# SaeedRahmani/AV-Simulation-at-Intersections

Hardware: AMD Instinct MI355X
Metric: MPC steps/sec (batch x horizon) at N=20 nu=2 (higher is better)
Workload: dtype f64

## Files before the change

### av-simulation-at-intersections_amd/_cabi.py

```python
from __future__ import annotations

import ctypes as C
import os

from .config import MPCConfig

_HERE = os.path.dirname(os.path.abspath(__file__))
LIB_PATH = os.environ.get("JSIM_LIB_PATH") or os.path.join(_HERE, "libjsim_mpc.so")
ABI_VERSION = 2


class JsimCfg(C.Structure):
    _fields_ = [
        ("T", C.c_int32), ("max_iter", C.c_int32),
        ("dt", C.c_double), ("dl", C.c_double), ("L", C.c_double),
        ("w_perp", C.c_double), ("w_para", C.c_double),
        ("R", C.c_double * 2), ("Rd", C.c_double * 2), ("Q_v_yaw", C.c_double * 2),
        ("Qf", C.c_double * 4), ("R_end", C.c_double * 2),
        ("max_dsteer", C.c_double), ("max_accel", C.c_double), ("max_decel", C.c_double),
        ("max_steer", C.c_double), ("max_speed", C.c_double), ("min_speed", C.c_double),
        ("min_ref_speed", C.c_double), ("goal_dis", C.c_double), ("stop_speed", C.c_double),
        ("nx", C.c_int32), ("reserved_", C.c_int32), ("jerk_weight", C.c_double),
    ]


EXPORTS = (
    "jsim_abi_version", "jsim_last_error", "jsim_mpc_create", "jsim_mpc_destroy", "jsim_mpc_set_paths",
    "jsim_mpc_step", "jsim_mpc_step_debug", "jsim_plant_step", "jsim_loop_advance", "jsim_mpc_run_ticks", "jsim_mpc_set_launch_order", "jsim_mpc_get_launch_order", "jsim_mpc_iter_totals",
    "jsim_loop_set_geometry", "jsim_loop_set_obstacle_geometry", "jsim_loop_predict_obstacles", "jsim_loop_pre_tick",
    "jsim_mpc_set_path_speed", "jsim_mpc_set_speed_cutoff", "jsim_mpc_update_cfg", "jsim_mpc_set_ego_config", "jsim_loop_obstacles",
    "jsim_mpc_xref_deviation_goal", "jsim_loop_run_scenario",
    "jsim_loop_set_groups", "jsim_loop_predict_egos", "jsim_loop_run_interacting",
    "jsim_loop_set_traffic", "jsim_loop_set_recorder", "jsim_loop_set_vehicle_shapes",
    "jsim_comm_unique_id", "jsim_comm_init", "jsim_mpc_gather", "jsim_comm_destroy", "jsim_plan_routes",
    "jsim_plan_routes_weighted", "jsim_score_trajectories", "jsim_loop_eval_reasons", "jsim_loop_eval_conflicts",
    "jsim_loop_eval_static", "jsim_loop_summarise_episodes", "jsim_loop_eval_cutoffs", "jsim_loop_fork_state", "jsim_loop_obstacles_at",
    "jsim_loop_eval_gaps",
)

_lib = None


class JsimError(RuntimeError):
    pass


def load() -> C.CDLL:
    global _lib
    if _lib is not None:
        return _lib
    if not os.path.exists(LIB_PATH):
        raise JsimError(
            f"{LIB_PATH} is missing: build it with `python __graft_entry__.py` (hipcc, gfx950). "
            "The MPC path is HIP-only; there is no CPU fallback.")
    lib = C.CDLL(LIB_PATH)
    vp, i32, i64, dbl = C.c_void_p, C.c_int32, C.c_int64, C.c_double
    lib.jsim_abi_version.restype = C.c_int
    lib.jsim_abi_version.argtypes = []
    lib.jsim_last_error.restype = C.c_char_p
    lib.jsim_last_error.argtypes = [vp]
    lib.jsim_mpc_create.restype = C.c_int
    lib.jsim_mpc_create.argtypes = [C.POINTER(JsimCfg), C.c_int, C.POINTER(vp)]
    lib.jsim_mpc_destroy.restype = None
    lib.jsim_mpc_destroy.argtypes = [vp]
    lib.jsim_mpc_set_paths.restype = C.c_int
    lib.jsim_mpc_set_paths.argtypes = [vp, vp, vp, vp, vp, i32]
    lib.jsim_mpc_step.restype = C.c_int
# ... 116 lines not shown
```

### av-simulation-at-intersections_amd/batched.py

```python
from __future__ import annotations

import ctypes as C
from typing import List, Optional, Sequence, Union

import numpy as np
import torch

from . import _cabi
from .config import MPCConfig
from .synth import pack_paths, smooth_yaw_inplace


def _ptr(t: Optional[torch.Tensor]):
    return None if t is None else C.c_void_p(t.data_ptr())


class BatchedMPC:

    def __init__(self, paths: Sequence[np.ndarray], path_id: Union[np.ndarray, Sequence[int]], dl: float,
                 L: float = 2.86, speed: Union[float, np.ndarray] = 30 / 3.6, dt: float = 0.2,
                 T: Optional[int] = None, config: Optional[MPCConfig] = None,
                 device: Union[str, torch.device] = "cuda:0", smooth: bool = True,
                 cv: Optional[Sequence[np.ndarray]] = None):
        self.lib = _cabi.load()
# ... 37 lines not shown
        self.path_id = torch.from_numpy(pid).to(dev)
        full = np.array([self.paths[i].shape[0] for i in pid], dtype=np.int32)
        self.path_len = torch.from_numpy(full.copy()).to(dev)
        self.full_len = torch.from_numpy(full).to(dev)
        sp = np.broadcast_to(np.asarray(speed, dtype=np.float64), (B,)).copy()
        self.speed = torch.from_numpy(sp).to(dev)
        MW = (8 * T + 31) // 32
        spec = [("target_ind", torch.int64, (B,)), ("oa", torch.float64, (B, T)), ("od", torch.float64, (B, T)),
                ("ox", torch.float64, (B, T + 1)), ("oy", torch.float64, (B, T + 1)), ("ov", torch.float64, (B, T + 1)),
                ("oyaw", torch.float64, (B, T + 1)), ("xref", torch.float64, (B, 4, T + 1)), ("di_ai", torch.float64, (B, 2)),
                ("active_mask", torch.int32, (B, MW)), ("status", torch.int32, (B,)), ("n_iter", torch.int32, (B,))]
        self._arena_layout = {}
        nbytes = 0
        for name, dt, shape in spec:
            n = int(np.prod(shape)) * torch.empty((), dtype=dt).element_size()
            self._arena_layout[name] = (nbytes, n, dt, shape)
            nbytes += (n + 7) & ~7
        self._arena = torch.zeros(max(nbytes, 8), dtype=torch.uint8, device=dev)
        for name, (o, n, dt, shape) in self._arena_layout.items():
            setattr(self, name, self._arena[o:o + n].view(dt).view(shape))

    def read_back(self) -> dict:
        host = self._arena.cpu().numpy()
        return {name: host[o:o + n].view(torch.empty((), dtype=dt).numpy().dtype).reshape(shape)
                for name, (o, n, dt, shape) in self._arena_layout.items()}

    def _upload_paths(self):
        cx, cy, cyaw, off = pack_paths(self.paths)
        self._path_off = off
        _cabi.check(self.lib.jsim_mpc_set_paths(self._ctx, cx.ctypes.data, cy.ctypes.data, cyaw.ctypes.data,
                                                off.ctypes.data, len(self.paths)), self._ctx, "jsim_mpc_set_paths")

    def set_path_len(self, path_len: Union[np.ndarray, torch.Tensor]):
        if isinstance(path_len, torch.Tensor):
            pl = path_len.to(device=self.device, dtype=torch.int32)
        else:
            pl = torch.from_numpy(np.ascontiguousarray(path_len, dtype=np.int32)).to(self.device)
        if pl.shape != (self.B,):
            raise ValueError("path_len must have shape [B]")
        if bool((pl < 1).any()) or bool((pl > self.full_len).any()):
            raise ValueError("path_len must satisfy 1 <= path_len[b] <= len(paths[path_id[b]])")
        self.path_len = pl.contiguous()

    def set_speed_cutoff(self, cutoff: Optional[Union[np.ndarray, torch.Tensor]]):
        if cutoff is None:
            self.cv_cut = None
            _cabi.check(self.lib.jsim_mpc_set_speed_cutoff(self._ctx, None), self._ctx, "jsim_mpc_set_speed_cutoff")
            return
# ... 109 lines not shown
```

### av-simulation-at-intersections_amd/csrc/mpc_step_reg.inc

```

template <int CTRL>
__device__ __forceinline__ double dpp_f64(double v)
{
    int lo = __double2loint(v), hi = __double2hiint(v);
    lo = __builtin_amdgcn_update_dpp(0, lo, CTRL, 0xf, 0xf, true);
    hi = __builtin_amdgcn_update_dpp(0, hi, CTRL, 0xf, 0xf, true);
    return __hiloint2double(hi, lo);
}
template <int CTRL>
__device__ __forceinline__ int dpp_i32(int v) { return __builtin_amdgcn_update_dpp(0, v, CTRL, 0xf, 0xf, true); }

#define DPP_QP_1032 0xB1
#define DPP_QP_2301 0x4E
#define DPP_ROW_HALF_MIRROR 0x141
#define DPP_ROW_MIRROR 0x140
#define DPP_ROW_SHR(n) (0x110 + (n))

__device__ __forceinline__ double wsum_dpp(double v)
{
    v += dpp_f64<DPP_QP_1032>(v);
    v += dpp_f64<DPP_QP_2301>(v);
    v += dpp_f64<DPP_ROW_HALF_MIRROR>(v);
    v += dpp_f64<DPP_ROW_MIRROR>(v);
    return (rdlane(v, 0) + rdlane(v, 16)) + (rdlane(v, 32) + rdlane(v, 48));
// ... 181 lines not shown
#endif
#ifndef JSIM_CHUNK_WAITS
#define JSIM_CHUNK_WAITS 15
#endif

#include "loop_pre_tick.inc"

struct PreK {
    PreP pre;
    const double2 *pred_cc_all;
    const double4 *pred_bc_all;
    long long *traj_idx;
    int *prev_len;
    int *path_len_out;
    int speed_cutoff;
    int *cut_io;
    int *col_flag;
    int *pre_status;
    TrafficP traffic;
};

enum { HB_SKIP = 0, HB_SCAN = 1, HB_HBUILD = 2, HB_JBUILD = 3, HB_EXIT = 4 };

__device__ __forceinline__ void jsim_spin_published(const double *val_lds)
{
    const unsigned addr = (unsigned)(__UINTPTR_TYPE__)(__attribute__((address_space(3))) const double *)val_lds;
    int v, cnt, cur;
    asm volatile("s_mov_b32 %1, 0\n"
                 "1:\n\t"
                 "ds_read_b32 %0, %3 offset:4\n\t"
                 "s_waitcnt lgkmcnt(0)\n\t"
                 "v_readfirstlane_b32 %2, %0\n\t"
                 "s_add_u32 %1, %1, 1\n\t"
                 "s_cmp_lg_u32 %2, 0xbff00000\n\t"
                 "s_cbranch_scc1 2f\n\t"
                 "s_cmp_lt_u32 %1, 0x400000\n\t"
                 "s_cbranch_scc1 1b\n"
                 "2:"
                 : "=&v"(v), "=&s"(cnt), "=&s"(cur)
                 : "v"(addr)
                 : "memory", "scc");
}

template <int T, int ROW>
__device__ __forceinline__ void jsim_h_tile_row(const double *tq, double *Hm, int lane, double dt)
{
    constexpr int N = 2 * T, LD = N + 1, TP = T + 2;
    const int kk = lane >> 4, cc = lane & 15;
    double c0[ROW + 1], c1[ROW + 1], p0[ROW + 1], p1[ROW + 1];
    int thr[ROW + 1];
    const bool isd_ = cc & 1;
    const int xrow = (kk < 2 ? (isd_ ? TQ_PB : TQ_PA) : TQ_ONE) * TP, yrow = (kk < 2 ? (isd_ ? TQ_PBP : TQ_PAP) : TQ_ONE) * TP;
    const int w0row = (kk == 0 ? TQ_QXX : kk == 1 ? TQ_QXY : kk == 2 ? TQ_QV : TQ_QYAW) * TP;
    const int w1row = (kk == 0 ? TQ_QXY : kk == 1 ? TQ_QYY : TQ_ZERO) * TP;
#pragma unroll
    for (int c = 0; c <= ROW; ++c) {
        const int col = 16 * c + cc;
        const bool vcol = col < N;
        const int s = vcol ? (col >> 1) : (T - 1);
        const double ks = tq[TQ_KT * TP + s];
        const double coef = vcol ? (isd_ ? ks : dt) : 0.0;
        const double c23 = !vcol ? 0.0 : (kk == 2 ? (isd_ ? 0.0 : dt) : (kk == 3 ? (isd_ ? ks : 0.0) : 0.0));
        c0[c] = kk < 2 ? coef : c23;
        c1[c] = kk < 2 ? coef : 0.0;
// ... 59 lines not shown
template <int T, bool PRE, int WPE, bool HELP = false>
__global__ __launch_bounds__(HELP ? 256 : 64) __attribute__((amdgpu_waves_per_eu(WPE, WPE)))
void mpc_step_reg_kernel(const KP Pin, const TickP K, const PreK Q)
{
    static_assert(!HELP || (WPE == 1 && (2 * T + 15) / 16 <= 4), "helpers: one wave per SIMD, one helper per tile row");
    KP P = Pin;
    if ((int)blockIdx.x >= Pin.B) return;
    const int ego = K.order ? K.order[blockIdx.x] : (int)blockIdx.x;
    if (Pin.pe) jsim_apply_ego_cfg(P, Pin.pe, ego, Pin.T, Pin.dt);
    constexpr int N = 2 * T, NR = 3 * T + 1, LD = N + 1, TP = T + 2, MW = (8 * T + 31) / 32;
    constexpr int NTILE = (N + 15) / 16;
    constexpr bool VS = NR >= 64;
    constexpr int NW = VS ? N : NR;
    static_assert(NW < 64, "register path needs 2T+1 lanes (3T+2 with resident speed rows)");
    constexpr int NP = N + 2;
    constexpr int CHW = VS ? 0 : HELP ? (JSIM_CHUNK_WAITS & ~2) : JSIM_CHUNK_WAITS;
    constexpr int LDC = N + 2, CCH = 16;
    constexpr bool LCA = VS || (WPE == 2 && T > 13);
    constexpr int HLN = LCA ? N * LDC : N * LD + N * LDC;
    constexpr int PREN = PRE ? (int)((sizeof(PreScratch) + 7) / 8) : 0;
    __shared__ __attribute__((aligned(16))) double HL[HLN > PREN ? HLN : PREN];
    double *const Hm = HL;
    constexpr bool HCLR = HELP && !LCA;
    double *const Lc = HL + (LCA ? 0 : N * LD);
    static_assert((N * LD) % 2 == 0, "Lc stays 16-byte aligned");
    __shared__ __attribute__((aligned(16))) double gsv[2 * N];
    __shared__ __attribute__((aligned(16))) double drow12[2 * NP];
    double *const drow = drow12, *const drow2 = drow12 + NP;
    __shared__ __attribute__((aligned(16))) double dzv[NP];
    __shared__ __attribute__((aligned(16))) double vzv[NP];
    __shared__ __attribute__((aligned(16))) double rdv[NP];
    __shared__ __attribute__((aligned(16))) double UV[VS ? 2 : NR + 5];
    constexpr int TQN = (TQ_COUNT * TP + 1) & ~1 ;
    constexpr int SPH = (T + 1) & ~1, SPN = VS ? T * SPH : 0;
    static_assert(!VS || (SPN >= NR + 5 || TQN + 3 * NP >= NR + 5), "uvec fits the shared area");
    __shared__ __attribute__((aligned(16))) double SCR[(TQN + 3 * NP > SPN) ? TQN + 3 * NP : SPN];
    double *const tq = SCR, *const invc = SCR + TQN, *const gvc = SCR + TQN + NP, *const wvc = SCR + TQN + 2 * NP;
    double *const spdump = SCR;
    double *const uvec = VS ? SCR : UV;
    __shared__ unsigned maskw[MW + 1];
    __shared__ int hb_cmd, hb_ilen;
    __shared__ __attribute__((aligned(16))) double Jx[HELP ? 64 * (N + 2) : 2];
    __shared__ long long hb_s0;
    __shared__ double hb_xy[2], hb_rd[HELP ? 12 : 2];
    __shared__ int hb_ri[HELP ? 12 : 2];

    const int lane0 = HELP ? (int)(threadIdx.x & 63) : (int)threadIdx.x;
    const int hwave = HELP ? __builtin_amdgcn_readfirstlane((int)(threadIdx.x >> 6)) : 0;
    if (P.pass > 0 && P.status[ego] != JSIM_OK) return;
    const int it_base = (P.pass > 0 && P.n_iter) ? P.n_iter[ego] : 0;
    int lane = lane0;

    const int pid = P.path_id[ego];
    const long long off = P.poff[pid];
    long long M = P.path_len[ego];
    long long pre_idx = 0;
    int pre_prev = -1, pre_col = 0, pre_st = JSIM_OK, Mfull = 0, pre_cut = -1;
    ObsSlice pre_obs = {0, 0};
    const double2 *pre_othr = nullptr;
    if (PRE) {
        pre_obs = traffic_slice(Q.traffic, ego, Q.pre.n_obs);
        pre_obs.first = uni(pre_obs.first); pre_obs.n = uni(pre_obs.n);
        if (Q.pre.othr) pre_othr = Q.pre.othr + pre_obs.first;
        pre_idx = Q.traj_idx[ego];
// ... 39 lines not shown
                    const double2 p0 = pp[k], p1 = pp[k + 192], p2 = pp[k + 384], p3 = pp[k + 576];
                    HB_INSERT_PT(p0, k) HB_INSERT_PT(p1, k + 192) HB_INSERT_PT(p2, k + 384) HB_INSERT_PT(p3, k + 576)
                }
                for (; k < ilen; k += 192) {
                    const double2 p0 = pp[k];
                    HB_INSERT_PT(p0, k)
                }
#undef HB_INSERT_PT
#pragma unroll
                for (int r = 0; r < 3; ++r) {
                    double v = b0;
                    int id = i0;
                    wargmin_fast(v, id);
                    if (lane0 == 0) { hb_rd[(hwave - 1) * 3 + r] = v; hb_ri[(hwave - 1) * 3 + r] = id; }
                    if (i0 == id) { b0 = b1; i0 = i1; b1 = b2; i1 = i2; b2 = INFINITY; i2 = 0x7fffffff; }
                }
            } else if (cmd == HB_HBUILD) {
                if (hwave == 1 && NTILE > 1) jsim_h_tile_row<T, 1>(tq, Hm, lane0, dt);
                else if (hwave == 2 && NTILE > 2) jsim_h_tile_row<T, 2>(tq, Hm, lane0, dt);
                else if (hwave == 3 && NTILE > 3) jsim_h_tile_row<T, 3>(tq, Hm, lane0, dt);
                if (hwave == 3) { const double gi = jsim_g_own<T>(tq, lane0, dt); if (lane0 < N) gvc[lane0] = gi; }
            } else if (cmd == HB_JBUILD && hwave == 1) {
                double Jr[N];
#define JSIM_J_WAIT(n_) jsim_spin_published(&invc[(n_) - 1])
#include "mpc_step_reg_j.inc"
#undef JSIM_J_WAIT
#pragma unroll
                for (int j = 0; j < N; j += 2) *(double2 *)&Jx[lane0 * (N + 2) + j] = double2{Jr[j], Jr[j + 1]};
            } else if (cmd == HB_JBUILD && HCLR) {
                for (int e = (hwave - 2) * 64 + lane0; e < N * LD; e += 128) Hm[e] = 0.0;
                if (hwave == 2 && lane0 < N) { gsv[2 * lane0] = 1.0; gsv[2 * lane0 + 1] = 0.0; }
                if (hwave == 3 && lane0 < 2) { drow[N + lane0] = 0.0; drow2[N + lane0] = 0.0; dzv[N + lane0] = 0.0; vzv[N + lane0] = 0.0; }
            }
            __syncthreads();
        }
    }
    double wtan;
    {
        double dc = (P.smax < wd_t) ? P.smax : wd_t;
        dc = (-P.smax > dc) ? -P.smax : dc;
        wtan = tan(dc);
    }
    for (int tk = 0; tk < K.n_ticks; ++tk) {
    if (WPE == 2) {
        sx = uni(sx); sy = uni(sy); sv = uni(sv); syaw = uni(syaw); di_prev = uni(di_prev); ai_last = uni(ai_last);
        goal_xy.x = uni(goal_xy.x); goal_xy.y = uni(goal_xy.y); s0 = uni64(s0); age = uni(age);
    }
#define LANE_FENCE() do { lane = lane0; asm volatile("" : "+v"(lane)); __builtin_assume(lane >= 0 && lane < 64); } while (0)
    LANE_FENCE();
    if (PRE) {
        PreScratch &W = *reinterpret_cast<PreScratch *>(HL);
        PreP pre = Q.pre;
        pre.n_obs = pre_obs.n;
        const PreOut o = jsim_pre_tick_ego(pre, Q.pred_cc_all + ((size_t)tk * Q.pre.n_obs + pre_obs.first) * Q.pre.n_steps * 2,
                                           Q.pred_bc_all + (size_t)tk * Q.pre.n_obs + pre_obs.first, pre_othr, W, lane, ego,
                                           off, Mfull, sx, sy, sv, pre_idx, pre_prev);
        pre_st = o.status;
        if (o.status == JSIM_OK) {
            pre_idx = o.idx; pre_col = o.col;
            if (Q.speed_cutoff) pre_cut = o.path_len; else M = o.path_len;
        }
        pre_prev = Q.speed_cutoff ? Mfull : (int)M;
        LDS_SYNC();
        LANE_FENCE();
    }
// ... 277 lines not shown
                        const double hv = 2.0 * acc[a][b][r];
                        Hm[row * LD + col] = hv;
                        if (a != b) Hm[col * LD + row] = hv;
                    }
                }
    }
    LDS_SYNC();
    STAMP(5);
    LANE_FENCE();
    double A[N];
    {
        const int i = lane < N ? lane : 0;
        const int t = i >> 1, c = i & 1;
        const double Rt = (tq[TQ_REND * TP + t] != 0.0) ? (c ? P.Re1 : P.Re0) : (c ? P.R1 : P.R0);
        const double rdc = 2.0 * (c ? P.Rd1 : P.Rd0);
        const int nd = (T >= 2) ? ((t == 0 || t == T - 1) ? 1 : 2) : 0;
        if (lane < N) {
            Hm[i * LD + i] += 2.0 * Rt + nd * rdc;
            if (i + 2 < N) Hm[i * LD + i + 2] -= rdc;
            if (i >= 2) Hm[i * LD + i - 2] -= rdc;
        }
        LDS_SYNC();
#pragma unroll
        for (int j = 0; j < N; ++j) A[j] = Hm[i * LD + j];
    }
    if (P.dbg_g && lane < N) P.dbg_g[(size_t)ego * N + lane] = gi_own;
    if (P.dbg_H && lane < N) {
        double *Hd = P.dbg_H + (size_t)ego * N * N + (size_t)lane * N;
#pragma unroll
        for (int j = 0; j < N; ++j) Hd[j] = A[j];
    }
    const double gmax = wmax_dpp(fabs(gi_own));

    if (lane < N) gvc[lane] = gi_own;
    STAMP(6);
    LANE_FENCE();
    if (HELP) {
        if (lane < N) invc[lane] = -1.0;
        if (lane == 0) hb_cmd = HB_JBUILD;
        __syncthreads();
    }
    {
        JSIM_OPAQUE_ZERO(zc_);
        const double *const LcC = Lc + zc_;
        double inv, tmul;
        {
            if (lane < N) Lc[lane] = A[0];
            double ck = rdlane(A[0], 0);
            if (!(ck > 0.0)) ck = 1e-300;
            inv = fast_rsqrt(ck);
            tmul = A[0] * (inv * inv);
        }
#pragma unroll
        for (int k = 0; k < N; ++k) {
            LDS_SYNC();
            const int j0 = k & ~1;
            const int nch = (N - j0 + CCH - 1) / CCH;
            double2 cb[2][CCH / 2];
#pragma unroll
            for (int j = j0; j < j0 + CCH && j < N; j += 2) cb[0][(j - j0) / 2] = *(const double2 *)&LcC[k * LDC + j];
            if (HELP) __builtin_amdgcn_fence(__ATOMIC_RELEASE, "wavefront");
            if (lane == k) invc[k] = inv;
            const double tk = tmul;
            if (k + 1 < N) {
                JSIM_STAGE();
                if (!(k & 1)) JSIM_PIN_PAIR(cb[0][0]);
                const double cn = ((k + 1) & 1) ? cb[0][(k + 1 - j0) / 2].y : cb[0][(k + 1 - j0) / 2].x;
                A[k + 1] = fma(-tk, cn, A[k + 1]);
                JSIM_PIN(A[k + 1]);
                if (lane >= k + 1 && lane < N) Lc[(k + 1) * LDC + lane] = A[k + 1];
                double ck = rdlane(A[k + 1], k + 1);
                if (!(ck > 0.0)) ck = 1e-300;
                inv = fast_rsqrt(ck);
                tmul = A[k + 1] * (inv * inv);
            }
#pragma unroll
            for (int c = 0; c < nch; ++c) {
                const int h = j0 + c * CCH;
                if (c + 1 < nch) {
#pragma unroll
                    for (int j = h + CCH; j < h + 2 * CCH && j < N; j += 2) cb[(c + 1) & 1][(j - h - CCH) / 2] = *(const double2 *)&LcC[k * LDC + j];
                }
                if ((CHW & 1) && k + 1 < N) jsim_chunk_wait((c + 1 < nch ? ((h + 2 * CCH < N ? h + 2 * CCH : N) - (h + CCH)) / 2 : 0) + (c == 0 ? 2 : 0));
                JSIM_STAGE();
#pragma unroll
                for (int j = h; j < h + CCH && j < N; j += 2) {
                    const double2 c2 = cb[c & 1][(j - h) / 2];
                    if (j > k + 1) { A[j] = fma(-tk, c2.x, A[j]); JSIM_PIN(A[j]); }
                    if (j + 1 > k + 1) { A[j + 1] = fma(-tk, c2.y, A[j + 1]); JSIM_PIN(A[j + 1]); }
                }
                JSIM_STAGE();
            }
        }
    }
    LDS_SYNC();

    STAMP(7);
    LANE_FENCE();
    double Jr[N];
    if (!HELP) {
#define JSIM_J_WAIT(n_) do { } while (0)
#include "mpc_step_reg_j.inc"
#undef JSIM_J_WAIT
    } else {
        __syncthreads();
        hp = 3;
#pragma unroll
        for (int j = 0; j < N; j += 2) { const double2 v2 = *(const double2 *)&Jx[lane * (N + 2) + j]; Jr[j] = v2.x; Jr[j + 1] = v2.y; }
    }
    LDS_SYNC();

    STAMP(8);
    LANE_FENCE();
    double val = 0.0;
    {
        double v0 = 0.0, v1 = 0.0;
        JSIM_OPAQUE_ZERO(zw_);
        const double *const wvW = wvc + zw_;
#pragma unroll
        for (int h = 0; h < N; h += CCH) {
            double2 wb[CCH / 2];
#pragma unroll
            for (int j = h; j < h + CCH && j < N; j += 2) wb[(j - h) / 2] = *(const double2 *)&wvW[j];
            JSIM_STAGE();
#pragma unroll
            for (int j = h; j < h + CCH && j < N; j += 2) {
                v0 = fma(-Jr[j], wb[(j - h) / 2].x, v0);
                v1 = fma(-Jr[j + 1], wb[(j - h) / 2].y, v1);
            }
// ... 465 lines not shown
        }
        if (failed) { status = JSIM_INFEASIBLE; break; }
    }
#undef JSIM_SEARCH
#undef JSIM_SEARCH_A
#undef JSIM_SEARCH_B1
#undef JSIM_SEARCH_B2
#undef JSIM_SEARCH_C

    STAMP(10);
#ifdef JSIM_STAMPS
    if (P.dbg_clk && lane == 0)
        for (int i_ = 0; i_ < 8; ++i_) P.dbg_clk[(size_t)P.B * 16 + (size_t)ego * 8 + i_] = gclk[i_];
#endif
    LANE_FENCE();
    if (status != JSIM_OK) {
        if (tl) { P.oa[(size_t)ego * T + lane] = 0.0; P.od[(size_t)ego * T + lane] = 0.0; }
        wa_t = 0.0; wd_t = 0.0; wtan = 0.0; s0 = tind;
        if (P.amask && lane < MW) P.amask[(size_t)ego * MW + lane] = 0u;
        if (lane == 0) {
            P.status[ego] = status;
            P.target_ind[ego] = tind;
            if (P.n_iter) P.n_iter[ego] = it_base + iters;
            if (K.work) K.work[ego] += (unsigned)iters;
            if (K.iters) K.iters[ego] += (unsigned long long)iters;
        }
        break;
    }
    if (lane < MW) maskw[lane] = 0u;
    if (lane < (VS ? N : NR)) uvec[lane] = val;
    if (VS) {
        const bool evl = lane < N && !(lane & 1);
        const double vsp = fma(dt, wincscan_dpp(evl ? val : 0.0, lane), sv);
        if (evl) uvec[N + (lane >> 1) + 1] = vsp;
        if (lane == 0) uvec[N] = sv;
    }
    if (P.dbg_lam)
        for (int e = lane; e < 8 * T; e += 64) P.dbg_lam[(size_t)ego * 8 * T + e] = 0.0;
    LDS_SYNC();
    {
        const double thr = JSIM_ACT_TOL * fmax(1.0, gmax);
        if (lane < q) {
            if (lam > thr) atomicOr(&maskw[actid >> 5], 1u << (actid & 31));
            if (P.dbg_lam) P.dbg_lam[(size_t)ego * 8 * T + actid] = lam;
        }
        LDS_SYNC();
        if (P.amask && lane < MW) P.amask[(size_t)ego * MW + lane] = maskw[lane];
    }
    {
// ... 7 lines not shown
        const double yt = syaw + wexscan_dpp(kt * dl_, lane);
        const double xt = sx + wexscan_dpp(fma(al, vt, fma(be, yt, ccx)), lane);
        const double yy = sy + wexscan_dpp(fma(alp, vt, fma(bep, yt, ccy)), lane);
        if (tl) { P.oa[(size_t)ego * T + lane] = a; P.od[(size_t)ego * T + lane] = dl_; }
        wa_t = a; wd_t = dl_; s0 = tind;
        if (K.advance || tk + 1 < K.n_ticks) {
            double dc = (P.smax < dl_) ? P.smax : dl_;
            dc = (-P.smax > dc) ? -P.smax : dc;
            wtan = tan(dc);
        }
        a0n = uvec[0]; d0n = uvec[1];
        if (lane <= T) {
            const size_t o = (size_t)ego * (T + 1) + lane;
            if (P.ox) P.ox[o] = xt;
            if (P.oy) P.oy[o] = yy;
            if (P.ov) P.ov[o] = vt;
            if (P.oyaw) P.oyaw[o] = yt;
        }
    }
    if (lane == 0) {
        P.status[ego] = JSIM_OK;
        P.target_ind[ego] = tind;
        if (P.n_iter) P.n_iter[ego] = it_base + iters;
        if (K.work) K.work[ego] += (unsigned)iters;
        if (K.iters) K.iters[ego] += (unsigned long long)iters;
    }
    STAMP(11);
    } while (0);
    if (HELP)
        for (; hp < 3; ++hp) {
            if (lane0 == 0) hb_cmd = HB_SKIP;
            __syncthreads();
            __syncthreads();
        }

    if (K.advance) {
        double di = di_prev, ai;
        if (status == JSIM_OK) { di = d0n; ai = a0n; }
        else ai = P.amin;
        di_prev = di;
        ai_last = ai;
        if (K.hist && lane == 0) {
            const int k = hist_base + tk;
            if (k < K.hist_cap) { K.hist[((size_t)k * P.B + ego) * 2] = di; K.hist[((size_t)k * P.B + ego) * 2 + 1] = ai; }
        }
        if (K.rec && lane == 0 && *K.tick + tk < K.rec_cap)
            jsim_rec_store_dev(K.rec, *K.tick + tk, P.B, ego,
                               status == JSIM_OK ? jsim_xref_deviation(P.pxy[off + s0], P.pyaw[off + s0], sx, sy) : __builtin_nan(""));
        double dc = (P.smax < di) ? P.smax : di;
// ... 18 lines not shown
        const bool done = (isgoal && fabs(sv) <= K.stop_speed) || (age + 1 >= K.max_age);
        if (K.rec && lane == 0) {
            const int k = *K.tick + tk;
            if (k < K.rec_cap)
                jsim_rec_store(K.rec, K.rec_flags, k, P.B, ego, sx, sy, syaw, sv, di, ai,
                               (status == JSIM_OK ? 0 : JSIM_REC_FAILED) | (isgoal && fabs(sv) <= K.stop_speed ? JSIM_REC_GOAL : 0) |
                                   (age + 1 >= K.max_age ? JSIM_REC_AGE : 0));
        }
        if (done) {
            sx = K.x0_spawn[4 * ego]; sy = K.x0_spawn[4 * ego + 1]; sv = K.x0_spawn[4 * ego + 2]; syaw = K.x0_spawn[4 * ego + 3];
            s0 = K.target_spawn[ego];
            wa_t = 0.0; wd_t = 0.0; wtan = 0.0; di_prev = 0.0; ai_last = 0.0; age = 0;
            if (PRE) { pre_idx = 0; pre_prev = -1; }
            if (tl) { P.oa[(size_t)ego * T + lane] = 0.0; P.od[(size_t)ego * T + lane] = 0.0; }
            if (lane == 0) {
                P.target_ind[ego] = s0;
                if (K.n_respawn) atomicAdd(K.n_respawn, 1ull);
            }
        } else {
            age += 1;
        }
    }
    LDS_SYNC();
    }
    if (HELP) {
        if (lane0 == 0) hb_cmd = HB_EXIT;
        __syncthreads();
    }
    if (K.advance && lane == 0) {
        K.x0w[4 * ego] = sx; K.x0w[4 * ego + 1] = sy; K.x0w[4 * ego + 2] = sv; K.x0w[4 * ego + 3] = syaw;
        K.di_ai[2 * ego] = di_prev;
        K.di_ai[2 * ego + 1] = ai_last;
        K.age[ego] = age;
    }
    if (PRE && lane == 0) {
        Q.traj_idx[ego] = pre_idx;
        Q.prev_len[ego] = pre_prev;
        if (Q.speed_cutoff) Q.cut_io[ego] = pre_cut; else Q.path_len_out[ego] = (int)M;
        Q.col_flag[ego] = pre_col;
        Q.pre_status[ego] = pre_st;
    }
}
```

### av-simulation-at-intersections_amd/csrc/mpc_step_reg4.inc

```

__host__ __device__ constexpr int jsim_tile_wave4(int ntile, int a)
{
    return ntile == 5 ? (a == 0 || a == 4 ? 0 : a) : (a & 3);
}

__device__ __forceinline__ double pair_swap(double v)
{
    double r = dpp_f64<DPP_QP_1032>(v);
    asm volatile("" : "+v"(r));
    return r;
}

#ifndef JSIM_REG4_MINW
#define JSIM_REG4_MINW 2
#endif

template <int T, bool PRE>
__global__ __launch_bounds__(256, JSIM_REG4_MINW) void mpc_step_reg4_kernel(const KP P, const TickP K, const PreK Q)
{
    constexpr int N = 2 * T, NH = T, NR = 3 * T + 1, LD = N + 2, TP = T + 2, MW = (8 * T + 31) / 32, NP = N + 2;
    constexpr int NTILE = (N + 15) / 16;
    constexpr int G1 = 31, G2 = 61;
    constexpr int S2 = 64 + (N - G2);
    constexpr int SW = S2 + T + 1;
// ... 62 lines not shown
        Mfull = (int)(gp(Pv.poff)[pid + 1] - off);
        if (Q.speed_cutoff) pre_cut = Q.cut_io[ego];
    }
    const double speed = uni(gp(Pv.speed)[ego]);
    const double dt = uni((double)Pv.dt);
#define tl (lane < T)
    long long s0 = uni64(gp(Pv.target_ind)[ego]);
    double sx = gp(Pv.x0)[4 * ego + 0], sy = gp(Pv.x0)[4 * ego + 1], sv = gp(Pv.x0)[4 * ego + 2], syaw = gp(Pv.x0)[4 * ego + 3];
#define WS_SET(a_, d_) do { if (wave == 0 && tl) { wsv[0][lane] = (a_); wsv[1][lane] = (d_); } } while (0)
#define WS_TAN(d_, out_) do { const double sm_ = Pv.smax; double dc_ = (sm_ < (d_)) ? sm_ : (d_); dc_ = (-sm_ > dc_) ? -sm_ : dc_; out_ = tan(dc_); } while (0)
    {
        double wt0 = 0.0;
        if (wave == 0 && tl) { const double od0 = gp(Pv.od)[(size_t)ego * T + lane]; WS_TAN(od0, wt0); }
        WS_SET(gp(Pv.oa)[(size_t)ego * T + lane], wt0);
    }
    __syncthreads();
    double di_prev = advance ? gp(Kv.di_ai)[2 * ego] : 0.0;
    double ai_last = advance ? gp(Kv.di_ai)[2 * ego + 1] : 0.0;
    int age = advance ? uni(gp(Kv.age)[ego]) : 0;
    const int hist_base = (advance && (Kv.hist || Kv.rec)) ? uni(*gp(Kv.tick)) : 0;
    double2 goal_xy = double2{0.0, 0.0};
    if (advance) { const jsim_d2v gq = ((JSIM_GAS const jsim_d2v *)Pv.pxy)[gp(Pv.poff)[pid + 1] - 1]; goal_xy = double2{uni(gq.x), uni(gq.y)}; }

    for (int tk = 0; tk < n_ticks; ++tk) {
#define LANE_FENCE4() do { unsigned ones_ = ~0u; asm volatile("" : "+s"(ones_)); gl = (wave << 6) | (int)__builtin_amdgcn_mbcnt_hi(ones_, __builtin_amdgcn_mbcnt_lo(ones_, 0u)); asm volatile("" : "+v"(gl)); __builtin_assume(gl >= 0 && gl < 256); lane = gl & 63; } while (0)
    LANE_FENCE4();
    sx = uni(sx); sy = uni(sy); sv = uni(sv); syaw = uni(syaw); di_prev = uni(di_prev); ai_last = uni(ai_last);
    s0 = uni64(s0); M = uni64(M); age = uni(age);
    if (PRE) {
        PreScratch &W = *reinterpret_cast<PreScratch *>(Hm);
        PreP pre = Q.pre;
        pre.n_obs = pre_obs.n;
        const PreOut o = jsim_pre_tick_ego<true>(pre, Q.pred_cc_all + ((size_t)tk * Q.pre.n_obs + pre_obs.first) * Q.pre.n_steps * 2,
                                           Q.pred_bc_all + (size_t)tk * Q.pre.n_obs + pre_obs.first, pre_othr, W, lane, ego,
                                           off, Mfull, sx, sy, sv, pre_idx, pre_prev);
        pre_st = o.status;
        if (o.status == JSIM_OK) {
            pre_idx = o.idx; pre_col = o.col;
            if (Q.speed_cutoff) pre_cut = o.path_len; else M = o.path_len;
        }
        pre_prev = Q.speed_cutoff ? Mfull : (int)M;
        BLOCK_SYNC();
        LANE_FENCE4();
    }
    double a0n = 0.0, d0n = 0.0;
    int status = JSIM_OK;
// ... 989 lines not shown
                    if (slot == dslot) abits &= ~(1u << dbit);
                    JSIM_PIN(abits);
                }
                GSTAMP(7);
            }
        }
        if (failed) { status = JSIM_INFEASIBLE; break; }
    }

#ifdef JSIM_STAMPS
    if (Pv.dbg_clk && gl == 0)
        for (int i_ = 0; i_ < 8; ++i_) Pv.dbg_clk[(size_t)Pv.B * 16 + (size_t)ego * 8 + i_] = gclk[i_];
#endif
    LANE_FENCE4();
    STAMP2(10);
    if (status != JSIM_OK) {
        if (wave == 0 && tl) { gp(Pv.oa)[(size_t)ego * T + lane] = 0.0; gp(Pv.od)[(size_t)ego * T + lane] = 0.0; }
        WS_SET(0.0, 0.0); s0 = tind;
        if (Pv.amask && gl < MW) gp(Pv.amask)[(size_t)ego * MW + gl] = 0u;
        if (gl == 0) {
            gp(Pv.status)[ego] = status;
            gp(Pv.target_ind)[ego] = tind;
            if (Pv.n_iter) gp(Pv.n_iter)[ego] = it_base + iters;
            if (Kv.work) gp(Kv.work)[ego] += (unsigned)iters;
            if (Kv.iters) gp(Kv.iters)[ego] += (unsigned long long)iters;
        }
        break;
    }
    if (gl < MW) maskw[gl] = 0u;
    {
        const int slot_ = gl >> 1;
        if (!(gl & 1)) {
            int jr_ = -1;
            if (slot_ < G1) jr_ = slot_;
            else if (slot_ > G1 && slot_ < G2 + 1) jr_ = slot_ - 1;
            else if (slot_ >= 64 && slot_ < S2) jr_ = slot_ - 3;
            if (jr_ >= 0) uvec[jr_] = val;
            if (slot_ >= S2 && slot_ < SW) uvec[N + slot_ - S2] = val;
        }
    }
    if (Pv.dbg_lam)
        for (int e = gl; e < 8 * T; e += 256) Pv.dbg_lam[(size_t)ego * 8 * T + e] = 0.0;
    BLOCK_SYNC();
    {
        const double thr = JSIM_ACT_TOL * fmax(1.0, gmax);
        if (wave == 0) {
            if (lane < q) {
                if (lam0 > thr) atomicOr(&maskw[act0 >> 5], 1u << (act0 & 31));
                if (Pv.dbg_lam) Pv.dbg_lam[(size_t)ego * 8 * T + act0] = lam0;
// ... 13 lines not shown
        if (tl) { a = uvec[2 * lane]; dl_ = uvec[2 * lane + 1]; }
        const double vt = lane <= T ? uvec[N + lane] : sv;
        const double yt = syaw + wexscan_dpp(kt * dl_, lane);
        const double xt = sx + wexscan_dpp(fma(al, vt, fma(be, yt, ccx)), lane);
        const double yy = sy + wexscan_dpp(fma(alp, vt, fma(bep, yt, ccy)), lane);
        if (wave == 0 && tl) { gp(Pv.oa)[(size_t)ego * T + lane] = a; gp(Pv.od)[(size_t)ego * T + lane] = dl_; }
        double tn = 0.0;
        if (advance || tk + 1 < n_ticks) WS_TAN(dl_, tn);
        p_tn = rdlane(tn, 0);
        WS_SET(a, tn); s0 = tind;
        a0n = uvec[0]; d0n = uvec[1];
        if (wave == 0 && lane <= T) {
            const size_t o = (size_t)ego * (T + 1) + lane;
            if (Pv.ox) gp(Pv.ox)[o] = xt;
            if (Pv.oy) gp(Pv.oy)[o] = yy;
            if (Pv.ov) gp(Pv.ov)[o] = vt;
            if (Pv.oyaw) gp(Pv.oyaw)[o] = yt;
        }
    }
    if (gl == 0) {
        gp(Pv.status)[ego] = JSIM_OK;
        gp(Pv.target_ind)[ego] = tind;
        if (Pv.n_iter) gp(Pv.n_iter)[ego] = it_base + iters;
        if (Kv.work) gp(Kv.work)[ego] += (unsigned)iters;
            if (Kv.iters) gp(Kv.iters)[ego] += (unsigned long long)iters;
    }
    STAMP2(11);
    } while (0);

    if (advance) {
        double di = di_prev, ai;
        if (status == JSIM_OK) { di = d0n; ai = a0n; }
        else ai = Pv.amin;
        di_prev = di;
        ai_last = ai;
        if (Kv.hist && gl == 0) {
            const int k = hist_base + tk;
            if (k < Kv.hist_cap) { gp(Kv.hist)[((size_t)k * Pv.B + ego) * 2] = di; gp(Kv.hist)[((size_t)k * Pv.B + ego) * 2 + 1] = ai; }
        }
        if (Kv.rec && gl == 0 && hist_base + tk < Kv.rec_cap) {
            const jsim_d2v rq = ((JSIM_GAS const jsim_d2v *)Pv.pxy)[off + s0];
            jsim_rec_store_dev(gp(Kv.rec), hist_base + tk, Pv.B, ego,
                               status == JSIM_OK ? jsim_xref_deviation(double2{rq.x, rq.y}, gp(Pv.pyaw)[off + s0], sx, sy)
                                                 : __builtin_nan(""));
        }
        double dc = (Pv.smax < di) ? Pv.smax : di;
        dc = (-Pv.smax > dc) ? -Pv.smax : dc;
        double cy_ = p_cs, sy_ = p_sn;
        if (!p_sc) { cy_ = cos(syaw); sy_ = sin(syaw); }
// ... 12 lines not shown
        const bool done = uni((int)(goal || aged)) != 0;
        if (Kv.rec && gl == 0) {
            const int k = hist_base + tk;
            if (k < Kv.rec_cap)
                jsim_rec_store(gp(Kv.rec), gp(Kv.rec_flags), k, Pv.B, ego, sx, sy, syaw, sv, di, ai,
                               (status == JSIM_OK ? 0 : JSIM_REC_FAILED) | (goal ? JSIM_REC_GOAL : 0) | (aged ? JSIM_REC_AGE : 0));
        }
        if (done) {
            sx = gp(Kv.x0_spawn)[4 * ego]; sy = gp(Kv.x0_spawn)[4 * ego + 1]; sv = gp(Kv.x0_spawn)[4 * ego + 2]; syaw = gp(Kv.x0_spawn)[4 * ego + 3];
            s0 = gp(Kv.target_spawn)[ego];
            WS_SET(0.0, 0.0); di_prev = 0.0; ai_last = 0.0; age = 0;
            if (PRE) { pre_idx = 0; pre_prev = -1; }
            if (wave == 0 && tl) { gp(Pv.oa)[(size_t)ego * T + lane] = 0.0; gp(Pv.od)[(size_t)ego * T + lane] = 0.0; }
            if (gl == 0) {
                gp(Pv.target_ind)[ego] = s0;
                if (Kv.n_respawn) atomicAdd(Kv.n_respawn, 1ull);
            }
        } else {
            age += 1;
        }
    }
    BLOCK_SYNC();
    }
    if (advance && gl == 0) {
        gp(Kv.x0w)[4 * ego] = sx; gp(Kv.x0w)[4 * ego + 1] = sy; gp(Kv.x0w)[4 * ego + 2] = sv; gp(Kv.x0w)[4 * ego + 3] = syaw;
        gp(Kv.di_ai)[2 * ego] = di_prev;
        gp(Kv.di_ai)[2 * ego + 1] = ai_last;
        gp(Kv.age)[ego] = age;
    }
    if (PRE && gl == 0) {
        Q.traj_idx[ego] = pre_idx;
        Q.prev_len[ego] = pre_prev;
        if (Q.speed_cutoff) Q.cut_io[ego] = pre_cut; else Q.path_len_out[ego] = (int)M;
        Q.col_flag[ego] = pre_col;
        Q.pre_status[ego] = pre_st;
    }
#undef LANE_FENCE4
#undef WS_SET
#undef WS_TAN
#undef tl
#undef SLOT_OF_ROW
#undef SLOTMAP4
}
```

### include/jsim_mpc.h

```cpp
#ifndef JSIM_MPC_H
#define JSIM_MPC_H

#include <stddef.h>
#include <stdint.h>

#ifdef __cplusplus
extern "C" {
#endif

#define JSIM_ABI_VERSION 2
#define JSIM_MAX_T 48

typedef struct jsim_cfg {
    int32_t T;
    int32_t max_iter;
    double dt, dl, L;
    double w_perp, w_para;
    double R[2], Rd[2], Q_v_yaw[2];
    double Qf[4];
    double R_end[2];
    double max_dsteer;
    double max_accel, max_decel;
    double max_steer, max_speed, min_speed;
    double min_ref_speed;
    double goal_dis, stop_speed;
    int32_t nx;
    int32_t reserved_;
    double jerk_weight;
} jsim_cfg;

typedef struct jsim_ctx jsim_ctx;

enum { JSIM_OK = 0, JSIM_INFEASIBLE = 1, JSIM_NEAREST_ANOMALY = 2 };

int jsim_abi_version(void);
const char *jsim_last_error(const jsim_ctx *ctx);

int jsim_mpc_create(const jsim_cfg *cfg, int device_id, jsim_ctx **out);
void jsim_mpc_destroy(jsim_ctx *ctx);

int jsim_mpc_set_paths(jsim_ctx *ctx, const double *cx, const double *cy, const double *cyaw,
                       const int64_t *path_off , int32_t n_paths);

int jsim_mpc_step(jsim_ctx *ctx, int32_t B, const double *x0, const int32_t *path_id,
                  const int32_t *path_len, const double *speed, int64_t *target_ind, double *oa,
                  double *od, double *ox, double *oy, double *ov, double *oyaw, double *xref,
                  uint32_t *active_mask, int32_t *status, int32_t *n_iter, void *stream);

int jsim_mpc_step_debug(jsim_ctx *ctx, int32_t B, const double *x0, const int32_t *path_id,
                        const int32_t *path_len, const double *speed, int64_t *target_ind, double *oa,
                        double *od, double *ox, double *oy, double *ov, double *oyaw, double *xref,
                        uint32_t *active_mask, int32_t *status, int32_t *n_iter, double *xbar,
                        int64_t *ref_idx, double *H, double *g, double *lam, void *stream);

int jsim_plant_step(jsim_ctx *ctx, int32_t B, double *x0, const double *oa, const double *od,
                    const int32_t *status, double *di_ai, void *stream);
// ... 149 lines not shown
```

Before: 5.075 million.

## Split Cholesky factor between main wave and helper wavefront, batch iteration counters

The dense Cholesky factorisation of the N×N Hessian is split so that the main wave factors only the leading NS columns. A helper wavefront applies the rank updates from those published columns to the trailing block and then factors that block itself, so the two run concurrently. The helper's spin-wait now has a timeout and reports a new status code, which Python checks on read-back. Per-ego work and iteration counter updates to global memory are accumulated in a register and written once after the tick loop. This adds cross-wave synchronisation complexity and a risk of timeouts or extra LDS traffic.

Result: faster. 5.178 million (median of 6 runs) (+2.0%).

```diff
diff --git a/av-simulation-at-intersections_amd/_cabi.py b/av-simulation-at-intersections_amd/_cabi.py
--- a/av-simulation-at-intersections_amd/_cabi.py
+++ b/av-simulation-at-intersections_amd/_cabi.py
@@ -43,6 +43,16 @@
 
 class JsimError(RuntimeError):
     pass
+
+
+STATUS_OK, STATUS_INFEASIBLE, STATUS_NEAREST_ANOMALY, STATUS_NO_PATH, STATUS_HELPER_TIMEOUT = 0, 1, 2, 3, 4
+
+
+def check_status(status, what: str) -> None:
+    bad = [int(b) for b in (status == STATUS_HELPER_TIMEOUT).nonzero()[0]]
+    if bad:
+        raise JsimError(f"{what}: status {STATUS_HELPER_TIMEOUT} (JSIM_HELPER_TIMEOUT) on ego(s) {bad[:8]}"
+                        f"{' ..' if len(bad) > 8 else ''}: a helper wavefront gave up waiting for a column of the factor")
 
 
 def load() -> C.CDLL:
diff --git a/av-simulation-at-intersections_amd/batched.py b/av-simulation-at-intersections_amd/batched.py
--- a/av-simulation-at-intersections_amd/batched.py
+++ b/av-simulation-at-intersections_amd/batched.py
@@ -83,8 +83,10 @@
 
     def read_back(self) -> dict:
         host = self._arena.cpu().numpy()
-        return {name: host[o:o + n].view(torch.empty((), dtype=dt).numpy().dtype).reshape(shape)
-                for name, (o, n, dt, shape) in self._arena_layout.items()}
+        out = {name: host[o:o + n].view(torch.empty((), dtype=dt).numpy().dtype).reshape(shape)
+               for name, (o, n, dt, shape) in self._arena_layout.items()}
+        _cabi.check_status(out["status"], "BatchedMPC.read_back")
+        return out
 
     def _upload_paths(self):
         cx, cy, cyaw, off = pack_paths(self.paths)
diff --git a/av-simulation-at-intersections_amd/csrc/mpc_step_reg.inc b/av-simulation-at-intersections_amd/csrc/mpc_step_reg.inc
--- a/av-simulation-at-intersections_amd/csrc/mpc_step_reg.inc
+++ b/av-simulation-at-intersections_amd/csrc/mpc_step_reg.inc
@@ -227,11 +227,12 @@
 
 enum { HB_SKIP = 0, HB_SCAN = 1, HB_HBUILD = 2, HB_JBUILD = 3, HB_EXIT = 4 };
 
-__device__ __forceinline__ void jsim_spin_published(const double *val_lds)
+__device__ __forceinline__ int jsim_spin_published(const double *val_lds, int tmo)
 {
     const unsigned addr = (unsigned)(__UINTPTR_TYPE__)(__attribute__((address_space(3))) const double *)val_lds;
+    const int cnt0 = __builtin_amdgcn_readfirstlane(tmo) ? 0x3fffff : 0;
     int v, cnt, cur;
-    asm volatile("s_mov_b32 %1, 0\n"
+    asm volatile("s_mov_b32 %1, %4\n"
                  "1:\n\t"
                  "ds_read_b32 %0, %3 offset:4\n\t"
                  "s_waitcnt lgkmcnt(0)\n\t"
@@ -243,8 +244,9 @@
                  "s_cbranch_scc1 1b\n"
                  "2:"
                  : "=&v"(v), "=&s"(cnt), "=&s"(cur)
-                 : "v"(addr)
+                 : "v"(addr), "s"(cnt0)
                  : "memory", "scc");
+    return cur == (int)0xbff00000;
 }
 
 template <int T, int ROW>
@@ -350,6 +352,8 @@
     __shared__ __attribute__((aligned(16))) double HL[HLN > PREN ? HLN : PREN];
     double *const Hm = HL;
     constexpr bool HCLR = HELP && !LCA;
+    constexpr bool SPLIT = HCLR;
+    constexpr int NS = SPLIT ? ((N / 2) & ~1) : N;
     double *const Lc = HL + (LCA ? 0 : N * LD);
     static_assert((N * LD) % 2 == 0, "Lc stays 16-byte aligned");
     __shared__ __attribute__((aligned(16))) double gsv[2 * N];
@@ -368,6 +372,7 @@
     double *const uvec = VS ? SCR : UV;
     __shared__ unsigned maskw[MW + 1];
     __shared__ int hb_cmd, hb_ilen;
+    __shared__ int hb_tmo;
     __shared__ __attribute__((aligned(16))) double Jx[HELP ? 64 * (N + 2) : 2];
     __shared__ long long hb_s0;
     __shared__ double hb_xy[2], hb_rd[HELP ? 12 : 2];
@@ -453,15 +458,78 @@
                 if (hwave == 3) { const double gi = jsim_g_own<T>(tq, lane0, dt); if (lane0 < N) gvc[lane0] = gi; }
             } else if (cmd == HB_JBUILD && hwave == 1) {
                 double Jr[N];
-#define JSIM_J_WAIT(n_) jsim_spin_published(&invc[(n_) - 1])
+                int tmo = 0;
+#define JSIM_J_WAIT(n_) do { if (!SPLIT || (n_) == 1 || !((n_) & 1)) tmo |= jsim_spin_published(&invc[(SPLIT && (n_) + 1 <= N ? (n_) + 1 : (n_)) - 1], tmo); } while (0)
 #include "mpc_step_reg_j.inc"
 #undef JSIM_J_WAIT
 #pragma unroll
                 for (int j = 0; j < N; j += 2) *(double2 *)&Jx[lane0 * (N + 2) + j] = double2{Jr[j], Jr[j + 1]};
-            } else if (cmd == HB_JBUILD && HCLR) {
-                for (int e = (hwave - 2) * 64 + lane0; e < N * LD; e += 128) Hm[e] = 0.0;
-                if (hwave == 2 && lane0 < N) { gsv[2 * lane0] = 1.0; gsv[2 * lane0 + 1] = 0.0; }
-                if (hwave == 3 && lane0 < 2) { drow[N + lane0] = 0.0; drow2[N + lane0] = 0.0; dzv[N + lane0] = 0.0; vzv[N + lane0] = 0.0; }
+                if (tmo && lane0 == 0) hb_tmo = 1;
+            } else if (cmd == HB_JBUILD && SPLIT && hwave == 2) {
+                if constexpr (SPLIT) {
+#ifdef JSIM_STAMPS
+#define HSTAMP(i) do { if (P.dbg_clk && lane0 == 0) P.dbg_clk[(size_t)ego * 16 + (i)] = (long long)__builtin_readcyclecounter(); } while (0)
+#else
+#define HSTAMP(i) do { } while (0)
+#endif
+                HSTAMP(12);
+                double A2[N - NS];
+                {
+                    const int i = lane0 < N ? lane0 : 0;
+#pragma unroll
+                    for (int j = NS; j < N; ++j) A2[j - NS] = Hm[i * LD + j];
+                    JSIM_STAGE();
+                    for (int e = lane0; e < N * LD / 2; e += 64) *(double2 *)&Hm[2 * e] = double2{0.0, 0.0};
+                }
+                int tmo = 0;
+                {
+                    JSIM_OPAQUE_ZERO(zs_);
+                    const double *const LcS = Lc + zs_, *const invS = invc + zs_;
+                    const int i = lane0 < N ? lane0 : 0;
+                    double2 cs[2][2][(N - NS) / 2];
+                    double own[2][2], invs[2][2];
+#define JSIM_S_READ(b_, k_)                                                                                                    \
+    {                                                                                                                          \
+        tmo |= jsim_spin_published(&invc[(k_) + 1], tmo);                                                                      \
+        _Pragma("unroll") for (int c = 0; c < 2; ++c) {                                                                        \
+            _Pragma("unroll") for (int j = NS; j < N; j += 2) cs[b_][c][(j - NS) / 2] = *(const double2 *)&LcS[((k_) + c) * LDC + j]; \
+            own[b_][c] = LcS[((k_) + c) * LDC + i]; invs[b_][c] = invS[(k_) + c];                                              \
+        }                                                                                                                      \
+    }
+                    JSIM_S_READ(0, 0)
+#pragma unroll
+                    for (int k = 0; k < NS; k += 2) {
+                        if (k + 2 < NS) JSIM_S_READ(((k >> 1) + 1) & 1, k + 2)
+                        JSIM_STAGE();
+#pragma unroll
+                        for (int c = 0; c < 2; ++c) {
+                            const double tk = own[(k >> 1) & 1][c] * (invs[(k >> 1) & 1][c] * invs[(k >> 1) & 1][c]);
+#pragma unroll
+                            for (int j = NS; j < N; j += 2) {
+                                const double2 c2 = cs[(k >> 1) & 1][c][(j - NS) / 2];
+                                A2[j - NS] = fma(-tk, c2.x, A2[j - NS]); JSIM_PIN(A2[j - NS]);
+                                A2[j + 1 - NS] = fma(-tk, c2.y, A2[j + 1 - NS]); JSIM_PIN(A2[j + 1 - NS]);
+                            }
+                        }
+                        JSIM_STAGE();
+                    }
+#undef JSIM_S_READ
+                }
+                if (tmo && lane0 == 0) hb_tmo = 1;
+                HSTAMP(13);
+#define JSIM_CH_K0 NS
+#define JSIM_CH_KE N
+#define JSIM_CH_A(j_) A2[(j_) - NS]
+#include "mpc_step_reg_chol.inc"
+#undef JSIM_CH_K0
+#undef JSIM_CH_KE
+#undef JSIM_CH_A
+                HSTAMP(14);
+#undef HSTAMP
+                }
+            } else if (cmd == HB_JBUILD && HCLR && hwave == 3) {
+                if (lane0 < N) { gsv[2 * lane0] = 1.0; gsv[2 * lane0 + 1] = 0.0; }
+                if (lane0 < 2) { drow[N + lane0] = 0.0; drow2[N + lane0] = 0.0; dzv[N + lane0] = 0.0; vzv[N + lane0] = 0.0; }
             }
             __syncthreads();
         }
@@ -472,6 +540,7 @@
         dc = (-P.smax > dc) ? -P.smax : dc;
         wtan = tan(dc);
     }
+    unsigned it_sum = 0;
     for (int tk = 0; tk < K.n_ticks; ++tk) {
     if (WPE == 2) {
         sx = uni(sx); sy = uni(sy); sv = uni(sv); syaw = uni(syaw); di_prev = uni(di_prev); ai_last = uni(ai_last);
@@ -795,13 +864,13 @@
         }
         LDS_SYNC();
 #pragma unroll
-        for (int j = 0; j < N; ++j) A[j] = Hm[i * LD + j];
+        for (int j = 0; j < NS; ++j) A[j] = Hm[i * LD + j];
     }
     if (P.dbg_g && lane < N) P.dbg_g[(size_t)ego * N + lane] = gi_own;
     if (P.dbg_H && lane < N) {
         double *Hd = P.dbg_H + (size_t)ego * N * N + (size_t)lane * N;
 #pragma unroll
-        for (int j = 0; j < N; ++j) Hd[j] = A[j];
+        for (int j = 0; j < N; ++j) Hd[j] = j < NS ? A[j] : Hm[lane * LD + j];
     }
     const double gmax = wmax_dpp(fabs(gi_own));
 
@@ -810,62 +879,16 @@
     LANE_FENCE();
     if (HELP) {
         if (lane < N) invc[lane] = -1.0;
-        if (lane == 0) hb_cmd = HB_JBUILD;
+        if (lane == 0) { hb_tmo = 0; hb_cmd = HB_JBUILD; }
         __syncthreads();
     }
-    {
-        JSIM_OPAQUE_ZERO(zc_);
-        const double *const LcC = Lc + zc_;
-        double inv, tmul;
-        {
-            if (lane < N) Lc[lane] = A[0];
-            double ck = rdlane(A[0], 0);
-            if (!(ck > 0.0)) ck = 1e-300;
-            inv = fast_rsqrt(ck);
-            tmul = A[0] * (inv * inv);
-        }
-#pragma unroll
-        for (int k = 0; k < N; ++k) {
-            LDS_SYNC();
-            const int j0 = k & ~1;
-            const int nch = (N - j0 + CCH - 1) / CCH;
-            double2 cb[2][CCH / 2];
-#pragma unroll
-            for (int j = j0; j < j0 + CCH && j < N; j += 2) cb[0][(j - j0) / 2] = *(const double2 *)&LcC[k * LDC + j];
-            if (HELP) __builtin_amdgcn_fence(__ATOMIC_RELEASE, "wavefront");
-            if (lane == k) invc[k] = inv;
-            const double tk = tmul;
-            if (k + 1 < N) {
-                JSIM_STAGE();
-                if (!(k & 1)) JSIM_PIN_PAIR(cb[0][0]);
-                const double cn = ((k + 1) & 1) ? cb[0][(k + 1 - j0) / 2].y : cb[0][(k + 1 - j0) / 2].x;
-                A[k + 1] = fma(-tk, cn, A[k + 1]);
-                JSIM_PIN(A[k + 1]);
-                if (lane >= k + 1 && lane < N) Lc[(k + 1) * LDC + lane] = A[k + 1];
-                double ck = rdlane(A[k + 1], k + 1);
-                if (!(ck > 0.0)) ck = 1e-300;
-                inv = fast_rsqrt(ck);
-                tmul = A[k + 1] * (inv * inv);
-            }
-#pragma unroll
-            for (int c = 0; c < nch; ++c) {
-                const int h = j0 + c * CCH;
-                if (c + 1 < nch) {
-#pragma unroll
-                    for (int j = h + CCH; j < h + 2 * CCH && j < N; j += 2) cb[(c + 1) & 1][(j - h - CCH) / 2] = *(const double2 *)&LcC[k * LDC + j];
-                }
-                if ((CHW & 1) && k + 1 < N) jsim_chunk_wait((c + 1 < nch ? ((h + 2 * CCH < N ? h + 2 * CCH : N) - (h + CCH)) / 2 : 0) + (c == 0 ? 2 : 0));
-                JSIM_STAGE();
-#pragma unroll
-                for (int j = h; j < h + CCH && j < N; j += 2) {
-                    const double2 c2 = cb[c & 1][(j - h) / 2];
-                    if (j > k + 1) { A[j] = fma(-tk, c2.x, A[j]); JSIM_PIN(A[j]); }
-                    if (j + 1 > k + 1) { A[j + 1] = fma(-tk, c2.y, A[j + 1]); JSIM_PIN(A[j + 1]); }
-                }
-                JSIM_STAGE();
-            }
-        }
-    }
+#define JSIM_CH_K0 0
+#define JSIM_CH_KE NS
+#define JSIM_CH_A(j_) A[(j_)]
+#include "mpc_step_reg_chol.inc"
+#undef JSIM_CH_K0
+#undef JSIM_CH_KE
+#undef JSIM_CH_A
     LDS_SYNC();
 
     STAMP(7);
@@ -878,6 +901,14 @@
     } else {
         __syncthreads();
         hp = 3;
+        if (__builtin_amdgcn_readfirstlane(hb_tmo)) {
+            status = JSIM_HELPER_TIMEOUT;
+            if (lane == 0) {
+                P.status[ego] = status;
+                if (P.n_iter) P.n_iter[ego] = it_base;
+            }
+            break;
+        }
 #pragma unroll
         for (int j = 0; j < N; j += 2) { const double2 v2 = *(const double2 *)&Jx[lane * (N + 2) + j]; Jr[j] = v2.x; Jr[j + 1] = v2.y; }
     }
@@ -1389,9 +1420,8 @@
             P.status[ego] = status;
             P.target_ind[ego] = tind;
             if (P.n_iter) P.n_iter[ego] = it_base + iters;
-            if (K.work) K.work[ego] += (unsigned)iters;
-            if (K.iters) K.iters[ego] += (unsigned long long)iters;
-        }
+        }
+        it_sum += (unsigned)iters;
         break;
     }
     if (lane < MW) maskw[lane] = 0u;
@@ -1445,9 +1475,8 @@
         P.status[ego] = JSIM_OK;
         P.target_ind[ego] = tind;
         if (P.n_iter) P.n_iter[ego] = it_base + iters;
-        if (K.work) K.work[ego] += (unsigned)iters;
-        if (K.iters) K.iters[ego] += (unsigned long long)iters;
-    }
+    }
+    it_sum += (unsigned)iters;
     STAMP(11);
     } while (0);
     if (HELP)
@@ -1512,6 +1541,10 @@
         }
     }
     LDS_SYNC();
+    if (tk + 1 >= K.n_ticks && lane == 0) {
+        if (K.work) K.work[ego] += it_sum;
+        if (K.iters) K.iters[ego] += (unsigned long long)it_sum;
+    }
     }
     if (HELP) {
         if (lane0 == 0) hb_cmd = HB_EXIT;
diff --git a/av-simulation-at-intersections_amd/csrc/mpc_step_reg4.inc b/av-simulation-at-intersections_amd/csrc/mpc_step_reg4.inc
--- a/av-simulation-at-intersections_amd/csrc/mpc_step_reg4.inc
+++ b/av-simulation-at-intersections_amd/csrc/mpc_step_reg4.inc
@@ -108,6 +108,7 @@
     double2 goal_xy = double2{0.0, 0.0};
     if (advance) { const jsim_d2v gq = ((JSIM_GAS const jsim_d2v *)Pv.pxy)[gp(Pv.poff)[pid + 1] - 1]; goal_xy = double2{uni(gq.x), uni(gq.y)}; }
 
+    unsigned it_sum = 0;
     for (int tk = 0; tk < n_ticks; ++tk) {
 #define LANE_FENCE4() do { unsigned ones_ = ~0u; asm volatile("" : "+s"(ones_)); gl = (wave << 6) | (int)__builtin_amdgcn_mbcnt_hi(ones_, __builtin_amdgcn_mbcnt_lo(ones_, 0u)); asm volatile("" : "+v"(gl)); __builtin_assume(gl >= 0 && gl < 256); lane = gl & 63; } while (0)
     LANE_FENCE4();
@@ -1143,9 +1144,8 @@
             gp(Pv.status)[ego] = status;
             gp(Pv.target_ind)[ego] = tind;
             if (Pv.n_iter) gp(Pv.n_iter)[ego] = it_base + iters;
-            if (Kv.work) gp(Kv.work)[ego] += (unsigned)iters;
-            if (Kv.iters) gp(Kv.iters)[ego] += (unsigned long long)iters;
-        }
+        }
+        it_sum += (unsigned)iters;
         break;
     }
     if (gl < MW) maskw[gl] = 0u;
@@ -1205,9 +1205,8 @@
         gp(Pv.status)[ego] = JSIM_OK;
         gp(Pv.target_ind)[ego] = tind;
         if (Pv.n_iter) gp(Pv.n_iter)[ego] = it_base + iters;
-        if (Kv.work) gp(Kv.work)[ego] += (unsigned)iters;
-            if (Kv.iters) gp(Kv.iters)[ego] += (unsigned long long)iters;
-    }
+    }
+    it_sum += (unsigned)iters;
     STAMP2(11);
     } while (0);
 
@@ -1266,6 +1265,10 @@
     }
     BLOCK_SYNC();
     }
+    if (gl == 0) {
+        if (Kv.work) gp(Kv.work)[ego] += it_sum;
+        if (Kv.iters) gp(Kv.iters)[ego] += (unsigned long long)it_sum;
+    }
     if (advance && gl == 0) {
         gp(Kv.x0w)[4 * ego] = sx; gp(Kv.x0w)[4 * ego + 1] = sy; gp(Kv.x0w)[4 * ego + 2] = sv; gp(Kv.x0w)[4 * ego + 3] = syaw;
         gp(Kv.di_ai)[2 * ego] = di_prev;
diff --git a/av-simulation-at-intersections_amd/csrc/mpc_step_reg_chol.inc b/av-simulation-at-intersections_amd/csrc/mpc_step_reg_chol.inc
--- /dev/null
+++ b/av-simulation-at-intersections_amd/csrc/mpc_step_reg_chol.inc
@@ -0,0 +1,54 @@
+    {
+        constexpr int K0 = JSIM_CH_K0, KE = JSIM_CH_KE;
+        JSIM_OPAQUE_ZERO(zc_);
+        const double *const LcC = Lc + zc_;
+        double inv, tmul;
+        {
+            if (K0 == 0 ? lane < N : (lane >= K0 && lane < N)) Lc[K0 * LDC + lane] = JSIM_CH_A(K0);
+            double ck = rdlane(JSIM_CH_A(K0), K0);
+            if (!(ck > 0.0)) ck = 1e-300;
+            inv = fast_rsqrt(ck);
+            tmul = JSIM_CH_A(K0) * (inv * inv);
+        }
+#pragma unroll
+        for (int k = K0; k < KE; ++k) {
+            LDS_SYNC();
+            const int j0 = k & ~1;
+            const int nch = (KE - j0 + CCH - 1) / CCH;
+            double2 cb[2][CCH / 2];
+#pragma unroll
+            for (int j = j0; j < j0 + CCH && j < KE; j += 2) cb[0][(j - j0) / 2] = *(const double2 *)&LcC[k * LDC + j];
+            if (HELP) __builtin_amdgcn_fence(__ATOMIC_RELEASE, "wavefront");
+            if (lane == k) invc[k] = inv;
+            const double tk = tmul;
+            if (k + 1 < KE) {
+                JSIM_STAGE();
+                if (!(k & 1)) JSIM_PIN_PAIR(cb[0][0]);
+                const double cn = ((k + 1) & 1) ? cb[0][(k + 1 - j0) / 2].y : cb[0][(k + 1 - j0) / 2].x;
+                JSIM_CH_A(k + 1) = fma(-tk, cn, JSIM_CH_A(k + 1));
+                JSIM_PIN(JSIM_CH_A(k + 1));
+                if (lane >= k + 1 && lane < N) Lc[(k + 1) * LDC + lane] = JSIM_CH_A(k + 1);
+                double ck = rdlane(JSIM_CH_A(k + 1), k + 1);
+                if (!(ck > 0.0)) ck = 1e-300;
+                inv = fast_rsqrt(ck);
+                tmul = JSIM_CH_A(k + 1) * (inv * inv);
+            }
+#pragma unroll
+            for (int c = 0; c < nch; ++c) {
+                const int h = j0 + c * CCH;
+                if (c + 1 < nch) {
+#pragma unroll
+                    for (int j = h + CCH; j < h + 2 * CCH && j < KE; j += 2) cb[(c + 1) & 1][(j - h - CCH) / 2] = *(const double2 *)&LcC[k * LDC + j];
+                }
+                if ((CHW & 1) && k + 1 < KE) jsim_chunk_wait((c + 1 < nch ? ((h + 2 * CCH < KE ? h + 2 * CCH : KE) - (h + CCH)) / 2 : 0) + (c == 0 ? 2 : 0));
+                JSIM_STAGE();
+#pragma unroll
+                for (int j = h; j < h + CCH && j < KE; j += 2) {
+                    const double2 c2 = cb[c & 1][(j - h) / 2];
+                    if (j > k + 1) { JSIM_CH_A(j) = fma(-tk, c2.x, JSIM_CH_A(j)); JSIM_PIN(JSIM_CH_A(j)); }
+                    if (j + 1 > k + 1) { JSIM_CH_A(j + 1) = fma(-tk, c2.y, JSIM_CH_A(j + 1)); JSIM_PIN(JSIM_CH_A(j + 1)); }
+                }
+                JSIM_STAGE();
+            }
+        }
+    }
diff --git a/include/jsim_mpc.h b/include/jsim_mpc.h
--- a/include/jsim_mpc.h
+++ b/include/jsim_mpc.h
@@ -31,7 +31,7 @@
 
 typedef struct jsim_ctx jsim_ctx;
 
-enum { JSIM_OK = 0, JSIM_INFEASIBLE = 1, JSIM_NEAREST_ANOMALY = 2 };
+enum { JSIM_OK = 0, JSIM_INFEASIBLE = 1, JSIM_NEAREST_ANOMALY = 2, JSIM_HELPER_TIMEOUT = 4 };
 
 int jsim_abi_version(void);
 const char *jsim_last_error(const jsim_ctx *ctx);
```
